# SynthAIr/T-VQ-VAE-TrajGen

Hardware: AMD Instinct MI355X
Metric: stage1+stage2 train steps/sec on synthetic (B,C,T) trajectories, 1/2/4/8 GPU (higher is better)
Workload: dtype fp32; 1 GPU; stage1 VQ-VAE + stage2 MaskGIT joint train step, per-GPU batch (B=256,C=6,T=256), K=512, configs/config.yaml architecture; global_batch=256, seq_len=256, parallelism=dp1, launch=hipgraph

## Files before the change

### include/tvq.h

```cpp
#ifndef TVQ_H
#define TVQ_H
#include <stdint.h>

#ifdef __cplusplus
extern "C" {
#endif

#define TVQ_OK 0
#define TVQ_ERR_ARG -1
#define TVQ_ERR_LAUNCH -2

typedef void* tvq_stream_t;

const char* tvq_last_error(void);
int tvq_abi_version(void);
const char* tvq_source_hash(void);
const char* tvq_build_extra(void);
int tvq_counter_pool(int64_t device, int32_t* zeroed, int64_t n);
int tvq_counter_capture(int64_t begin);
int tvq_fill(float* p, int64_t n, float value, tvq_stream_t stream);
int tvq_fill_i64(int64_t* p, int64_t n, int64_t value, tvq_stream_t stream);
int tvq_fill2(float* p, float a, float* q, float b, tvq_stream_t stream);
int tvq_add_i64(int64_t* p, int64_t value, tvq_stream_t stream);
int tvq_sum4(const float* a, const float* b, const float* c, const float* d, float* out,
// ... 44 lines not shown
                     int32_t* sel, tvq_stream_t stream);

int tvq_vq_expire(const float* x, int64_t B, int64_t N, int64_t D, int64_t sB, int64_t sN,
                  int64_t sD, const int32_t* sel, const int64_t* seed_ptr, uint64_t offset,
                  const float* cluster_size, float threshold, int64_t K, float* embed,
                  int32_t* n_expired, tvq_stream_t stream);

int64_t tvq_vq_kmeans_workspace(int64_t M, int64_t K, int64_t D);
int tvq_vq_kmeans(const float* x, int64_t B, int64_t N, int64_t D, int64_t sB, int64_t sN,
                  int64_t sD, const int32_t* sel, int64_t K, int64_t iters, float* means,
                  float* bins, int32_t* workspace, tvq_stream_t stream);


int tvq_stft_encode(const float* x, int64_t B, int64_t C, int64_t T, float* raw, float* enc_l,
                    float* enc_h, float* tgt_l, float* tgt_h, tvq_stream_t stream);

int tvq_istft_decode(const float* h, int64_t B, int64_t C, int64_t W, int64_t band, int64_t Tout,
                     float* y, tvq_stream_t stream);
int tvq_istft_decode_bwd(const float* dy, int64_t B, int64_t C, int64_t W, int64_t band,
                         int64_t Tout, float* dh, tvq_stream_t stream);

int tvq_conv_out_width(int64_t Win, int64_t KW, int64_t SW, int64_t transposed);
int tvq_conv_config(int64_t halo);

int tvq_conv_packcache_begin(int64_t id, float* arena, int64_t cap_floats, tvq_stream_t stream);
int tvq_conv_packcache_end(void);
int tvq_conv_packcache_release(int64_t id);
int tvq_conv_packcache_pause(int64_t on);
int64_t tvq_conv_packcache_entries(void);

int tvq_conv_wgrad_defer_begin(void);
int tvq_conv_wgrad_defer_flush(tvq_stream_t stream);
int tvq_wgrad_defer_begin_stream(tvq_stream_t stream);
int tvq_conv_wgrad_defer_pause(int64_t paused);
int64_t tvq_conv_workspace(int64_t op, int64_t B, int64_t Ci, int64_t H, int64_t Wi, int64_t Co,
                           int64_t KH, int64_t KW, int64_t SW, int64_t replicate);
int tvq_conv2d_fwd(const float* x, int64_t B, int64_t Ci, int64_t H, int64_t Wi, const float* w,
                   const float* bias, int64_t Co, int64_t KH, int64_t KW, int64_t SW,
                   int64_t replicate, float* y, const float* residual, float drop_p,
                   const int64_t* seed_ptr, uint64_t offset, float* workspace,
                   tvq_stream_t stream);
int tvq_convT2d_fwd(const float* x, int64_t B, int64_t Ci, int64_t H, int64_t Wi, const float* w,
                    const float* bias, int64_t Co, int64_t KH, int64_t KW, int64_t SW, float* y,
                    const float* residual, float* workspace, tvq_stream_t stream);
int tvq_conv2d_fwd_bn_eval(const float* x, int64_t B, int64_t Ci, int64_t H, int64_t Wi,
                           const float* w, const float* bias, int64_t Co, int64_t KH, int64_t KW,
// ... 389 lines not shown
```

### t-vq-vae-trajgen_amd/csrc/tvq_conv.hip

```cpp
#include "tvq_conv_core.h"

namespace tvq {

static ConvConfig g_conv_cfg;
const ConvConfig& conv_config() { return g_conv_cfg; }

__global__ void replicate_fold_kernel(const float* __restrict__ dpad, int B, int C, int H, int W,
                                      int PH, int PW, float* __restrict__ dx) {
  const int Hp = H + 2 * PH, Wp = W + 2 * PW;
  const int64_t tot = (int64_t)B * C * H * W;
  for (int64_t i = blockIdx.x * (int64_t)blockDim.x + threadIdx.x; i < tot;
       i += (int64_t)gridDim.x * blockDim.x) {
    const int w = (int)(i % W);
    const int64_t t = i / W;
    const int h = (int)(t % H);
    const int64_t bc = t / H;
    const float* p = dpad + bc * Hp * Wp;
    const int hlo = h == 0 ? 0 : h + PH, hhi = h == H - 1 ? Hp - 1 : h + PH;
    const int wlo = w == 0 ? 0 : w + PW, whi = w == W - 1 ? Wp - 1 : w + PW;
    float s = 0.f;
    for (int hh = hlo; hh <= hhi; ++hh)
      for (int ww = wlo; ww <= whi; ++ww) s += p[hh * Wp + ww];
    dx[i] = s;
  }
// ... 52 lines not shown
  e.drop_scale = drop_p > 0.f ? 1.0f / (1.0f - drop_p) : 1.0f;
  e.seed_ptr = seed_ptr;
  e.offset = offset;
  return e;
}

extern "C" int tvq_conv_config(int64_t halo) {
  ConvConfig& c = g_conv_cfg;
  const int prev = c.halo | (c.t32 ? 0 : 8) | (c.t32_bk == 32 ? 16 : 0) |
                   (c.t32_bk == 16 ? 32 : 0) | (c.t32_nw == 4 ? 64 : 0) | (c.t32_n64 ? 128 : 0) |
                   (c.small ? 0 : 256) | (c.s2 ? 0 : 512) | (c.ws2 ? 0 : 1024) |
                   (c.n16 ? 0 : 2048);
  if (halo >= 0) {
    c.halo = (int)(halo & 7);
    c.t32 = (halo & 8) ? 0 : 1;
    c.t32_bk = (halo & 16) ? 32 : ((halo & 32) ? 16 : 64);
    c.t32_nw = (halo & 64) ? 4 : 12;
    c.t32_n64 = (halo & 128) ? 1 : 0;
    c.small = (halo & 256) ? 0 : 1;
    c.s2 = (halo & 512) ? 0 : 1;
    c.ws2 = (halo & 1024) ? 0 : 1;
    c.n16 = (halo & 2048) ? 0 : 1;
  }
  return prev;
}

extern "C" int tvq_conv_out_width(int64_t Win, int64_t KW, int64_t SW, int64_t transposed) {
  const int64_t PW = (KW - 1) / 2;
  return (int)(transposed ? (Win - 1) * SW - 2 * PW + KW : (Win + 2 * PW - KW) / SW + 1);
}

static ConvGeom geom_conv_fwd(int64_t B, int64_t Ci, int64_t H, int64_t Wi, int64_t Co, int64_t KH,
                              int64_t KW, int64_t SW) {
  const int Wo = tvq_conv_out_width(Wi, KW, SW, 0);
  return make_geom((int)B, (int)Ci, (int)H, (int)Wi, (int)Co, (int)H, Wo, (int)KH, (int)KW,
                   PH_OF(KH), PW_OF(KW), Ci * KH * KW, KH * KW);
}
static ConvGeom geom_convT_fwd(int64_t B, int64_t Ci, int64_t H, int64_t Wi, int64_t Co,
                               int64_t KH, int64_t KW, int64_t SW) {
  const int Wo = tvq_conv_out_width(Wi, KW, SW, 1);
  return make_geom((int)B, (int)Ci, (int)H, (int)Wi, (int)Co, (int)H, Wo, (int)KH, (int)KW,
                   PH_OF(KH), PW_OF(KW), KH * KW, Co * KH * KW);
}
static ConvGeom geom_conv_dgrad(int64_t B, int64_t Ci, int64_t H, int64_t Wi, int64_t Co,
                                int64_t KH, int64_t KW, int64_t SW, int64_t replicate) {
  const int Wo = tvq_conv_out_width(Wi, KW, SW, 0);
// ... 229 lines not shown
```

### t-vq-vae-trajgen_amd/csrc/tvq_conv_core.h

```cpp
#pragma once
#include "tvq_common.h"

namespace tvq {

struct FastDiv {
  uint32_t d;
  uint64_t magic;
  uint32_t shift;
};
static FastDiv make_fastdiv(uint32_t d) {
  FastDiv f;
  f.d = d;
  uint32_t s = 0;
  while ((1ull << s) < d) ++s;
  f.shift = 32 + s;
  f.magic = ((1ull << f.shift) + d - 1) / d;
  return f;
}
__device__ __forceinline__ uint32_t fdiv(uint32_t n, const FastDiv& f) {
  return (uint32_t)(((uint64_t)n * f.magic) >> f.shift);
}

struct ConvGeom {
  int B, C, Hin, Win;
// ... 249 lines not shown
    switch (kind) {                                                                      \
      case 0: M(GATHER_T, 3, 4, 2, false) break;                                         \
      case 1: M(GATHER_T, 3, 3, 1, false) break;                                         \
      case 2: M(GATHER_T, 1, 1, 1, false) break;                                         \
      case 3: M(GATHER_T, 1, 3, 1, false) break;                                         \
      case 4: M(GATHER_T, 1, 7, 1, false) break;                                         \
      case 5: M(GATHER_T, 1, 4, 2, false) break;                                         \
    }                                                                                    \
  }

#ifndef TVQ_T32_BK
#define TVQ_T32_BK 64
#endif
struct ConvConfig {
  int halo = 3;
  int t32 = 1;
  int t32_bk = TVQ_T32_BK;
  int t32_nw = 12;
  int t32_n64 = 0;
  int small = 1;
  int s2 = 1;
  int ws2 = 1;
  int n16 = 1;
};
const ConvConfig& conv_config();


const float* pack_weight(const float* wt, ConvGeom& g, int KK, float* ws, hipStream_t st);

int s2_kind(int mode, const ConvGeom& g);
int64_t s2_blocks(const ConvGeom& g);
void launch_s2(int k2, bool repl, const float* in, const float* wt, float* out, const ConvGeom& g,
               const Epi& e, hipStream_t st);
bool s2_fold_fits(const ConvGeom& g);
void launch_s2_fold(const float* in, const float* wt, float* dx, const ConvGeom& g, hipStream_t st);
bool ws2_fits(int64_t C, int64_t H, int64_t N, int64_t KH, int64_t KW, int64_t SW);
int64_t ws2_ws(int64_t B, int64_t C, int64_t Wo, int64_t N);
int ws2_launch(const float* G, const float* X, float* slab, int B, int C, int N, int Win, int Wo,
               int kcols, bool repl, hipStream_t st);

bool launch_small(int mode, int kind, bool repl, const float* in, const float* wt, float* out,
                  const ConvGeom& g, const Epi& e, hipStream_t st);
bool n16_geom_ok(int mode, int kind, const ConvGeom& g);
void launch_n16(int mode, int kind, const float* in, const float* wp, float* out,
                const ConvGeom& g, const Epi& e, hipStream_t st);
bool launch_halo(int mode, int kind, bool repl, const float* in, const float* wt, float* out,
// ... 19 lines not shown
```

### t-vq-vae-trajgen_amd/csrc/tvq_conv_s2.hip

```cpp
#include "tvq_conv_core.h"
#include "tvq_reduce.h"

namespace tvq {

constexpr int S2_SEG = 64;
constexpr int S2_XRF = 2 * S2_SEG + 2;
constexpr int S2_XRT = S2_SEG / 2 + 4;

__device__ __forceinline__ void s2_bn_stats_block(double (&s1)[4], double (&s2)[4], int nbase,
                                                  int N, double* __restrict__ part) {
  __shared__ double red[4][16][2];
  const int lane = threadIdx.x & 63, wid = threadIdx.x >> 6;
#pragma unroll
  for (int r = 0; r < 4; ++r)
#pragma unroll
    for (int o = 1; o < 16; o <<= 1) {
      s1[r] += __shfl_xor(s1[r], o, 64);
      s2[r] += __shfl_xor(s2[r], o, 64);
    }
  if ((lane & 15) == 0) {
#pragma unroll
    for (int r = 0; r < 4; ++r) {
      red[wid][nbase + r][0] = s1[r];
      red[wid][nbase + r][1] = s2[r];
    }
  }
  __syncthreads();
  const int t = threadIdx.x;
  if (t < 2 * N) {
    const int n = t >> 1, k = t & 1;
    part[((int64_t)n * gridDim.x + blockIdx.x) * 2 + k] =
        ((red[0][n][k] + red[1][n][k]) + red[2][n][k]) + red[3][n][k];
  }
}

template <bool REPL, int CS, bool POST = false, bool STATS = false>
__global__ __launch_bounds__(256) void conv_s2f_kernel(const float* __restrict__ in,
                                                       const float* __restrict__ wt,
                                                       float* __restrict__ out, ConvGeom g, Epi e) {
  constexpr int NS = 3 * CS, RS = 5;
  constexpr int XN = CS * RS * S2_XRF, XPER = (XN + 255) / 256;
  __shared__ float Xs[XN];
  const int tid = threadIdx.x, lane = tid & 63, r16 = lane & 15, g4 = lane >> 4;
  const int wid = __builtin_amdgcn_readfirstlane(tid >> 6);
  const int segs = (g.Wo + S2_SEG - 1) / S2_SEG;
  const int b = blockIdx.x / segs, w0 = (blockIdx.x - b * segs) * S2_SEG;
  float af[NS];
  const int nr = r16 < g.N ? r16 : 0;
#pragma unroll
  for (int s = 0; s < NS; ++s) {
    const int c = s / 3, kh = s - 3 * c;
    const int cc = c < g.C ? c : 0;
    af[s] = wt[nr * g.wsn + cc * g.wsc + (kh * 4 + g4) * g.wst];
  }
  const float* inb = in + (int64_t)b * g.C * g.Hin * g.Win;
  float xv[XPER];
  uint64_t okm = 0;
#pragma unroll
  for (int u = 0; u < XPER; ++u) {
    const int i = tid + 256 * u;
    const int ck = i / S2_XRF, j = i - ck * S2_XRF, c = ck / RS, r = ck - RS * c;
    int hi = r - 1, wi = 2 * w0 - g.opw + j;
    bool ok = i < XN && c < g.C;
    if (REPL) {
      hi = hi < 0 ? 0 : (hi >= g.Hin ? g.Hin - 1 : hi);
      wi = wi < 0 ? 0 : (wi >= g.Win ? g.Win - 1 : wi);
    } else {
      ok = ok && hi >= 0 && hi < g.Hin && wi >= 0 && wi < g.Win;
    }
    xv[u] = inb[ok ? ((int64_t)c * g.Hin + hi) * g.Win + wi : 0];
    okm |= (uint64_t)(ok ? 1 : 0) << u;
  }
#pragma unroll
  for (int u = 0; u < XPER; ++u) {
    const int i = tid + 256 * u;
    if (i < XN) Xs[i] = (okm >> u & 1) ? xv[u] : 0.f;
  }
  float bv[1][4];
  const int nbase = 4 * g4;
  epi_load_bias<1>(bv, e.bias, nbase, g.N);
  __syncthreads();
  floatx4 acc[3];
  const float* xb[3];
#pragma unroll
  for (int t = 0; t < 3; ++t) {
    const int tile = wid * 3 + t, h = tile >> 2, p0 = (tile & 3) * 16;
    xb[t] = Xs + h * S2_XRF + 2 * (p0 + r16) + g4;
    acc[t] = floatx4{0.f, 0.f, 0.f, 0.f};
  }
#pragma unroll
  for (int s = 0; s < NS; ++s) {
    const int c = s / 3, kh = s - 3 * c, off = (c * RS + kh) * S2_XRF;
#pragma unroll
    for (int t = 0; t < 3; ++t) acc[t] = mfma16x16x4(af[s], xb[t][off], acc[t]);
  }
  const uint64_t seed = e.drop_p > 0.f ? mix_seed(e.seed_ptr, e.offset) : 0ull;
  const int64_t hw = (int64_t)g.Hout * g.Wo;
  PostTile<1> pt;
  if constexpr (POST) epi_load_post<1>(pt, e, nbase, g.N);
#pragma unroll
  for (int t = 0; t < 3; ++t) {
    const int tile = wid * 3 + t, h = tile >> 2;
    const int wo = w0 + (tile & 3) * 16 + r16;
    const bool pv = wo < g.Wo;
    const floatx4 a[1] = {acc[t]};
    epi_store<1, POST>(out, e, seed, bv, a, ((int64_t)b * g.N * g.Hout + h) * g.Wo + (pv ? wo : 0),
                       hw, nbase, g.N, pv, false, &pt);
  }
  if constexpr (STATS) {
    double s1[4] = {0.0, 0.0, 0.0, 0.0}, s2[4] = {0.0, 0.0, 0.0, 0.0};
#pragma unroll
    for (int t = 0; t < 3; ++t) {
      const int tile = wid * 3 + t;
      if (w0 + (tile & 3) * 16 + r16 >= g.Wo) continue;
#pragma unroll
      for (int r = 0; r < 4; ++r) {
        const double v = (double)(acc[t][r] + bv[0][r]);
        s1[r] += v;
        s2[r] += v * v;
      }
    }
    s2_bn_stats_block(s1, s2, nbase, g.N, e.bn_part);
  }
}

template <int CS, int HO, bool FOLD = false, bool POST = false, bool STATS = false>
__global__ __launch_bounds__(256) void conv_s2t_kernel(const float* __restrict__ in,
                                                       const float* __restrict__ wt,
                                                       float* __restrict__ out, ConvGeom g, Epi e) {
  constexpr int NS = 6 * CS / 4, RS = 7;
  constexpr int XN = CS * RS * S2_XRT, XPER = (XN + 255) / 256;
  __shared__ float Xs[XN];
  const int tid = threadIdx.x, lane = tid & 63, r16 = lane & 15, g4 = lane >> 4;
  const int wid = __builtin_amdgcn_readfirstlane(tid >> 6);
  const int par = wid & 1, mb = wid >> 1;
  const int segs = (g.Wo + S2_SEG - 1) / S2_SEG;
  const int b = blockIdx.x / segs, w0 = (blockIdx.x - b * segs) * S2_SEG;
  const int m0 = w0 >> 1;
  float af[NS];
  int soff[NS];
  const int nr = r16 < g.N ? r16 : 0, q = (par + g.opw) & 1;
#pragma unroll
  for (int s = 0; s < NS; ++s) {
    const int k = 4 * s + g4, c = k / 6, rem = k - 6 * c, kh = rem >> 1, kw = q + 2 * (rem & 1);
    const int cc = c < g.C ? c : 0;
    af[s] = wt[nr * g.wsn + cc * g.wsc + (kh * 4 + kw) * g.wst];
    soff[s] = (c * RS - kh) * S2_XRT + ((par + g.opw - kw) >> 1);
  }
  const float* inb = in + (int64_t)b * g.C * g.Hin * g.Win;
  float xv[XPER];
  uint32_t okm = 0;
  static_assert(XPER <= 32, "staging mask");
#pragma unroll
  for (int u = 0; u < XPER; ++u) {
    const int i = tid + 256 * u;
    const int ck = i / S2_XRT, j = i - ck * S2_XRT, c = ck / RS, r = ck - RS * c;
    const int hi = r - 2, wi = m0 - 2 + j;
    const bool ok = i < XN && c < g.C && hi >= 0 && hi < g.Hin && wi >= 0 && wi < g.Win;
    xv[u] = inb[ok ? ((int64_t)c * g.Hin + hi) * g.Win + wi : 0];
    okm |= (uint32_t)(ok ? 1 : 0) << u;
  }
#pragma unroll
  for (int u = 0; u < XPER; ++u) {
    const int i = tid + 256 * u;
    if (i < XN) Xs[i] = (okm >> u & 1) ? xv[u] : 0.f;
  }
  float bv[1][4];
  const int nbase = 4 * g4;
  epi_load_bias<1>(bv, e.bias, nbase, g.N);
  __syncthreads();
  floatx4 acc[HO];
  const float* xb = Xs + (g.oph + 2) * S2_XRT + mb * 16 + r16 + 2;
#pragma unroll
  for (int h = 0; h < HO; ++h) acc[h] = floatx4{0.f, 0.f, 0.f, 0.f};
#pragma unroll
  for (int s = 0; s < NS; ++s)
#pragma unroll
    for (int h = 0; h < HO; ++h) acc[h] = mfma16x16x4(af[s], xb[h * S2_XRT + soff[s]], acc[h]);
  const int wo = w0 + 2 * (mb * 16 + r16) + par;
  if constexpr (FOLD) {
    static_assert(HO == 5, "fold: replicate canvas");
    __shared__ floatx4 ex[2][3][4];
    const int Wx = g.Wo - 2;
    floatx4 y[3] = {acc[0] + acc[1], acc[2], acc[3] + acc[4]};
    if (wo == 0 || wo == Wx + 1) {
#pragma unroll
      for (int h = 0; h < 3; ++h) ex[wo == 0 ? 0 : 1][h][g4] = y[h];
    }
    __syncthreads();
    if (wo == 1) {
#pragma unroll
      for (int h = 0; h < 3; ++h) y[h] = ex[0][h][g4] + y[h];
    } else if (wo == Wx) {
#pragma unroll
      for (int h = 0; h < 3; ++h) y[h] = y[h] + ex[1][h][g4];
    }
    const bool pv = wo >= 1 && wo <= Wx;
#pragma unroll
    for (int h = 0; h < 3; ++h)
#pragma unroll
      for (int r = 0; r < 4; ++r) {
        const int n = nbase + r;
        if (pv && n < g.N) out[(((int64_t)b * g.N + n) * 3 + h) * Wx + wo - 1] = y[h][r];
      }
    return;
  }
  const uint64_t seed = e.drop_p > 0.f ? mix_seed(e.seed_ptr, e.offset) : 0ull;
  const int64_t hw = (int64_t)g.Hout * g.Wo;
  const bool pv = wo < g.Wo;
  PostTile<1> pt;
  if constexpr (POST) epi_load_post<1>(pt, e, nbase, g.N);
#pragma unroll
  for (int h = 0; h < HO; ++h) {
    const floatx4 a[1] = {acc[h]};
    epi_store<1, POST>(out, e, seed, bv, a, ((int64_t)b * g.N * g.Hout + h) * g.Wo + (pv ? wo : 0),
                       hw, nbase, g.N, pv, false, &pt);
  }
  if constexpr (STATS) {
    double s1[4] = {0.0, 0.0, 0.0, 0.0}, s2[4] = {0.0, 0.0, 0.0, 0.0};
    if (pv) {
#pragma unroll
      for (int h = 0; h < HO; ++h)
#pragma unroll
        for (int r = 0; r < 4; ++r) {
          const double v = (double)(acc[h][r] + bv[0][r]);
          s1[r] += v;
          s2[r] += v * v;
        }
    }
    s2_bn_stats_block(s1, s2, nbase, g.N, e.bn_part);
  }
}

int s2_kind(int mode, const ConvGeom& g) {
  if (!conv_config().s2 || g.C > 16 || g.N > 16 || g.Hin != 3) return 0;
  if (mode == GATHER_F)
    return g.Hout == 3 && g.oph == 1 && g.opw >= 0 && g.opw <= 2 ? 1 : 0;
  if (g.opw < 0 || g.opw > 3) return 0;
  if (g.Hout == 3 && g.oph == 1) return 2;
  if (g.Hout == 5 && g.oph == 0) return 3;
  return 0;
}

int64_t s2_blocks(const ConvGeom& g) { return (int64_t)g.B * ((g.Wo + S2_SEG - 1) / S2_SEG); }

template <bool REPL>
static void launch_s2_r(int kind, const float* in, const float* wt, float* out, const ConvGeom& g,
                        const Epi& e, hipStream_t st) {
  const dim3 grid((unsigned)s2_blocks(g));
  const int cs = (g.C + 3) / 4;
  TVQ_PLAN("conv_s2%s cs%d hout%d%s", kind == 1 ? "f" : "t", 4 * cs, g.Hout,
           e.bn_part ? " bnstats" : "");
#define S2F(CSV)                                                                                \
  do {                                                                                          \
    if (e.bn_part)                                                                              \
      hipLaunchKernelGGL((conv_s2f_kernel<REPL, CSV, false, true>), grid, dim3(256), 0, st, in,  \
                         wt, out, g, e);                                                        \
    else if (e.bn_rv)                                                                           \
      hipLaunchKernelGGL((conv_s2f_kernel<REPL, CSV, true>), grid, dim3(256), 0, st, in, wt, out, \
                         g, e);                                                                 \
    else                                                                                        \
      hipLaunchKernelGGL((conv_s2f_kernel<REPL, CSV>), grid, dim3(256), 0, st, in, wt, out, g, e); \
  } while (0)
#define S2T(CSV, HOV)                                                                            \
  do {                                                                                           \
    if (e.bn_part)                                                                               \
      hipLaunchKernelGGL((conv_s2t_kernel<CSV, HOV, false, false, true>), grid, dim3(256), 0, st, \
                         in, wt, out, g, e);                                                     \
    else if (e.bn_rv)                                                                            \
      hipLaunchKernelGGL((conv_s2t_kernel<CSV, HOV, false, true>), grid, dim3(256), 0, st, in, wt, \
                         out, g, e);                                                             \
    else                                                                                         \
      hipLaunchKernelGGL((conv_s2t_kernel<CSV, HOV>), grid, dim3(256), 0, st, in, wt, out, g, e); \
  } while (0)
  if (kind == 1) {
    if (cs == 1) S2F(4); else if (cs == 2) S2F(8); else if (cs == 3) S2F(12); else S2F(16);
    return;
  }
  if (kind == 2) {
    if (cs == 1) S2T(4, 3); else if (cs == 2) S2T(8, 3); else if (cs == 3) S2T(12, 3); else S2T(16, 3);
  } else {
    if (cs == 1) S2T(4, 5); else if (cs == 2) S2T(8, 5); else if (cs == 3) S2T(12, 5); else S2T(16, 5);
  }
#undef S2F
#undef S2T
}
void launch_s2(int k2, bool repl, const float* in, const float* wt, float* out, const ConvGeom& g,
               const Epi& e, hipStream_t st) {
  if (repl) launch_s2_r<true>(k2, in, wt, out, g, e, st);
  else launch_s2_r<false>(k2, in, wt, out, g, e, st);
}

bool s2_fold_fits(const ConvGeom& g) {
  return s2_kind(GATHER_T, g) == 3 && g.Wo >= 4 && (g.Wo - 1) % S2_SEG != 0;
}
void launch_s2_fold(const float* in, const float* wt, float* dx, const ConvGeom& g,
                    hipStream_t st) {
  const dim3 grid((unsigned)s2_blocks(g));
  const Epi e = {nullptr, nullptr, 0.f, 1.f, nullptr, 0};
  const int cs = (g.C + 3) / 4;
  TVQ_PLAN("conv_s2t_fold cs%d", 4 * cs);
#define S2T(CSV) hipLaunchKernelGGL((conv_s2t_kernel<CSV, 5, true>), grid, dim3(256), 0, st, in, wt, dx, g, e)
  if (cs == 1) S2T(4); else if (cs == 2) S2T(8); else if (cs == 3) S2T(12); else S2T(16);
#undef S2T
}

constexpr int W2_T = 512, W2_GS = 3 * S2_SEG + 4, W2_KP = 2 * S2_XRF + 2 * S2_SEG + 8;
struct W2Geom {
  int B, C, N, Win, Wo, Kred, kcols, segs, spr, opw;
};

template <bool REPL, int CS>
__global__ __launch_bounds__(W2_T) void conv_wgrad_s2_kernel(const float* __restrict__ G,
                                                            const float* __restrict__ X,
                                                            float* __restrict__ slab, W2Geom g) {
  constexpr int RS = 5, XN = CS * RS * S2_XRF, XPER = (XN + W2_T - 1) / W2_T;
  constexpr int GN = 16 * 3 * S2_SEG, GPER = GN / W2_T;
  constexpr int KT = (12 * CS + 1 + 15) / 16, TPW = (KT + 3) / 4;
  constexpr int RED = 4 * TPW * 256;
  static_assert(XPER <= 32 && GN % W2_T == 0, "staging");
  __shared__ float Xs[XN > RED ? XN : RED];
  __shared__ float Gs[16 * W2_GS];
  __shared__ float K1[2 * W2_KP];
  const int tid = threadIdx.x, lane = tid & 63, r16 = lane & 15, g4 = lane >> 4;
  const int wid = __builtin_amdgcn_readfirstlane(tid >> 6);
  const int tg = wid & 3, ph = wid >> 2;
  const int nst = g.B * g.segs, z = blockIdx.x;
  const int s_begin = z * g.spr, s_end = min(nst, s_begin + g.spr);
  for (int i = tid; i < 2 * W2_KP; i += W2_T) K1[i] = i < W2_KP ? 1.f : 0.f;
  const float* bp[TPW];
#pragma unroll
  for (int t = 0; t < TPW; ++t) {
    const int kc = (tg + 4 * t) * 16 + r16;
    const int k = kc < g.Kred ? kc : 0, c = k / 12, rem = k - 12 * c, kh = rem >> 2;
    bp[t] = (kc < g.Kred ? Xs + (c * RS + kh) * S2_XRF + (rem & 3)
                         : (kc == g.Kred && g.kcols > g.Kred ? K1 : K1 + W2_KP)) + 2 * g4;
  }
  const float* ap = Gs + r16 * W2_GS + g4;
  float xv[XPER], gv[GPER];
  uint32_t okm = 0, gok = 0;
  auto load = [&](int s) {
    const int b = s / g.segs, w0 = (s - b * g.segs) * S2_SEG;
    const float* xb = X + (int64_t)b * g.C * 3 * g.Win;
#pragma unroll
    for (int u = 0; u < XPER; ++u) {
      const int i = tid + W2_T * u;
      const int ck = i / S2_XRF, j = i - ck * S2_XRF, c = ck / RS, r = ck - RS * c;
      int hi = r - 1, wi = 2 * w0 - g.opw + j;
      bool ok = i < XN && c < g.C;
      if (REPL) {
        hi = hi < 0 ? 0 : (hi > 2 ? 2 : hi);
        wi = wi < 0 ? 0 : (wi >= g.Win ? g.Win - 1 : wi);
      } else {
        ok = ok && hi >= 0 && hi < 3 && wi >= 0 && wi < g.Win;
      }
      xv[u] = xb[ok ? ((int64_t)c * 3 + hi) * g.Win + wi : 0];
      okm = u == 0 ? (ok ? 1u : 0u) : (okm | (ok ? 1u : 0u) << u);
    }
    const float* gb = G + (int64_t)b * g.N * 3 * g.Wo;
#pragma unroll
    for (int u = 0; u < GPER; ++u) {
      const int i = tid + W2_T * u;
      const int n = i / (3 * S2_SEG), p = i - n * (3 * S2_SEG), h = p / S2_SEG, w = w0 + p - h * S2_SEG;
      const bool ok = n < g.N && w < g.Wo;
      gv[u] = gb[ok ? ((int64_t)n * 3 + h) * g.Wo + w : 0];
      gok = u == 0 ? (ok ? 1u : 0u) : (gok | (ok ? 1u : 0u) << u);
    }
  };
  auto store = [&]() {
#pragma unroll
    for (int u = 0; u < XPER; ++u) {
      const int i = tid + W2_T * u;
      if (i < XN) Xs[i] = (okm >> u & 1u) ? xv[u] : 0.f;
    }
#pragma unroll
    for (int u = 0; u < GPER; ++u) {
      const int i = tid + W2_T * u;
      const int n = i / (3 * S2_SEG), p = i - n * (3 * S2_SEG);
      Gs[n * W2_GS + p] = (gok >> u & 1u) ? gv[u] : 0.f;
    }
  };
  floatx4 acc[TPW];
#pragma unroll
  for (int t = 0; t < TPW; ++t) acc[t] = floatx4{0.f, 0.f, 0.f, 0.f};
  if (s_begin < s_end) load(s_begin);
  for (int s = s_begin; s < s_end; ++s) {
    __syncthreads();
    store();
    __syncthreads();
    if (s + 1 < s_end) load(s + 1);
#pragma unroll
    for (int i = 0; i < 24; ++i) {
      const int p0 = 96 * ph + 4 * i, h = p0 / S2_SEG, w = p0 - h * S2_SEG;
      const float a = ap[p0];
      const int off = h * S2_XRF + 2 * w;
#pragma unroll
      for (int t = 0; t < TPW; ++t) acc[t] = mfma16x16x4(a, bp[t][off], acc[t]);
    }
  }
  __syncthreads();
  floatx4* red = reinterpret_cast<floatx4*>(Xs);
  if (ph == 1) {
#pragma unroll
    for (int t = 0; t < TPW; ++t) red[(tg * TPW + t) * 64 + lane] = acc[t];
  }
  __syncthreads();
  if (ph == 0) {
    float* sl = slab + (int64_t)z * g.N * g.kcols;
#pragma unroll
    for (int t = 0; t < TPW; ++t) {
      const floatx4 o = red[(tg * TPW + t) * 64 + lane];
      const int kc = (tg + 4 * t) * 16 + r16;
#pragma unroll
      for (int r = 0; r < 4; ++r) {
        const int n = 4 * g4 + r;
        const float v = acc[t][r] + o[r];
        if (n < g.N && kc < g.kcols) sl[(int64_t)n * g.kcols + kc] = v;
      }
    }
  }
// ... 39 lines not shown
```

### t-vq-vae-trajgen_amd/timevqvae/hip/_native.py

```python
import ctypes
import os
import threading

import torch

_HERE = os.path.dirname(os.path.abspath(__file__))
LIB_PATH = os.environ.get(
    "TVQ_HIP_LIB", os.path.join(os.path.dirname(os.path.dirname(_HERE)), "lib", "libtvq_hip.so"))

P = ctypes.c_void_p
I64 = ctypes.c_int64
I32 = ctypes.c_int
F32 = ctypes.c_float

SIGNATURES = {}
_lib = None
_lock = threading.Lock()


def sig(name, *argtypes, restype=I32):
    SIGNATURES[name] = (list(argtypes), restype)


CSRC = os.path.join(os.path.dirname(os.path.dirname(_HERE)), "csrc")
# ... 48 lines not shown
sig("tvq_vq_sqnorm", P, I64, I64, P, P)
sig("tvq_vq_assign_nblocks", I64, restype=I64)
sig("tvq_vq_assign", P, I64, I64, I64, I64, I64, I64, P, P, I64, I32, P, P, P, P, P)
sig("tvq_vq_stats_workspace", I64, I64, restype=I64)
sig("tvq_vq_stats", P, I64, I64, I64, I64, I64, I64, P, I64, P, P, P, P, P)
sig("tvq_vq_ema", P, P, I64, I64, F32, P, P, P)
sig("tvq_vq_finalize", P, P, I64, I64, F32, P, P, I64, P, P, I64, P, P)
sig("tvq_vq_backward", P, P, P, P, I64, I64, P, P)

U64 = ctypes.c_uint64
sig("tvq_vq_assign_svq", P, I64, I64, I64, I64, I64, I64, P, P, I64, I32, F32, P, P, U64, P, P, P,
    P, P)
sig("tvq_vq_assign_rows", P, I64, I64, I64, I64, I64, I64, P, P, I64, I32, F32, P, P, U64, P, P, P,
    P, P, P)
sig("tvq_vq_draw_rows", I64, I64, P, U64, P, P)
sig("tvq_vq_expire", P, I64, I64, I64, I64, I64, I64, P, P, U64, P, F32, I64, P, P, P)
sig("tvq_vq_kmeans_workspace", I64, I64, I64, restype=I64)
sig("tvq_vq_kmeans", P, I64, I64, I64, I64, I64, I64, P, I64, I64, P, P, P, P)
sig("tvq_stft_encode", P, I64, I64, I64, P, P, P, P, P, P)
sig("tvq_istft_decode", P, I64, I64, I64, I64, I64, P, P)
sig("tvq_istft_decode_bwd", P, I64, I64, I64, I64, I64, P, P)
sig("tvq_conv_out_width", I64, I64, I64, I64)
sig("tvq_conv_config", I64)
sig("tvq_conv_workspace", I64, I64, I64, I64, I64, I64, I64, I64, I64, I64, restype=I64)
sig("tvq_conv2d_fwd", P, I64, I64, I64, I64, P, P, I64, I64, I64, I64, I64, P, P, F32, P, U64, P, P)
sig("tvq_convT2d_fwd", P, I64, I64, I64, I64, P, P, I64, I64, I64, I64, P, P, P, P)
sig("tvq_conv2d_fwd_bn_eval", P, I64, I64, I64, I64, P, P, I64, I64, I64, I64, I64, I64, P, P, P, P,
    F32, P, P, P, P)
sig("tvq_convT2d_fwd_bn_eval", P, I64, I64, I64, I64, P, P, I64, I64, I64, I64, P, P, P, P, F32, P,
    P, P, P)
sig("tvq_conv2d_dgrad", P, I64, I64, I64, I64, P, I64, I64, I64, I64, I64, P, I64, P, P)
sig("tvq_convT2d_dgrad", P, I64, I64, I64, I64, P, I64, I64, I64, I64, P, I64, P, P)
sig("tvq_conv2d_wgrad", P, I64, I64, I64, I64, P, I64, I64, I64, I64, I64, I64, P, P, I64, P, P)
sig("tvq_convT2d_wgrad", P, I64, I64, I64, I64, P, I64, I64, I64, I64, I64, P, I64, P, P)
sig("tvq_channel_sum_workspace", I64, I64, I64, restype=I64)
sig("tvq_channel_sum", P, I64, I64, I64, P, I64, P, P)
sig("tvq_bn_workspace", I64, I64, I64, restype=I64)
sig("tvq_bn_train_fwd", P, I64, I64, I64, P, P, P, P, P, F32, F32, P, P, P, P, P, P, P)
sig("tvq_bn_eval_fwd", P, I64, I64, I64, P, P, P, P, F32, P, P, P, P)
sig("tvq_bn_bwd", P, P, I64, I64, I64, P, P, P, P, P, P, P, P, P, I64, P, P)
sig("tvq_snake_fwd", P, I64, I64, I64, P, P, P)
sig("tvq_snake_workspace", I64, I64, I64, restype=I64)
sig("tvq_snake_bwd", P, P, I64, I64, I64, P, P, P, P, I64, P, P)
sig("tvq_dropout_bwd", P, I64, F32, P, U64, P, P)
sig("tvq_resblock_workspace", I64, I64, I64, I64, restype=I64)
sig("tvq_resblock_saved_floats", I64, I64, I64, I64, restype=I64)
# ... 217 lines not shown
```

Baseline: 260.7 steps/s.

## Make stride-2 conv kernels persistent with double-buffered async global-to-LDS staging

Converts the stride-2 forward and transposed conv kernels from one-segment-per-block into persistent blocks that walk several segments. The next segment is prefetched into a double-buffered dynamic-LDS ring with global_load_lds while the current one runs MFMA. Halo padding rows are no longer staged: only the three real input rows are loaded, and out-of-range rows point at shared zero rows or are clamped through pointer selection. The same row trimming is applied to the stride-2 wgrad kernel. The per-block segment count is controlled by a new s2_cap knob. The aim is to hide load latency and cut redundant staging, at the cost of more LDS, lower occupancy and ring synchronisation overhead.

```diff
diff --git a/include/tvq.h b/include/tvq.h
--- a/include/tvq.h
+++ b/include/tvq.h
@@ -90,6 +90,7 @@
 
 int tvq_conv_out_width(int64_t Win, int64_t KW, int64_t SW, int64_t transposed);
 int tvq_conv_config(int64_t halo);
+int tvq_conv_s2_cap(int64_t cap);
 
 int tvq_conv_packcache_begin(int64_t id, float* arena, int64_t cap_floats, tvq_stream_t stream);
 int tvq_conv_packcache_end(void);
diff --git a/t-vq-vae-trajgen_amd/csrc/tvq_conv.hip b/t-vq-vae-trajgen_amd/csrc/tvq_conv.hip
--- a/t-vq-vae-trajgen_amd/csrc/tvq_conv.hip
+++ b/t-vq-vae-trajgen_amd/csrc/tvq_conv.hip
@@ -98,6 +98,12 @@
     c.ws2 = (halo & 1024) ? 0 : 1;
     c.n16 = (halo & 2048) ? 0 : 1;
   }
+  return prev;
+}
+
+extern "C" int tvq_conv_s2_cap(int64_t cap) {
+  const int prev = g_conv_cfg.s2_cap;
+  if (cap >= 0) g_conv_cfg.s2_cap = cap > (1 << 30) ? (1 << 30) : (int)cap;
   return prev;
 }
 
diff --git a/t-vq-vae-trajgen_amd/csrc/tvq_conv_core.h b/t-vq-vae-trajgen_amd/csrc/tvq_conv_core.h
--- a/t-vq-vae-trajgen_amd/csrc/tvq_conv_core.h
+++ b/t-vq-vae-trajgen_amd/csrc/tvq_conv_core.h
@@ -295,6 +295,7 @@
   int s2 = 1;
   int ws2 = 1;
   int n16 = 1;
+  int s2_cap = 0;
 };
 const ConvConfig& conv_config();
 
diff --git a/t-vq-vae-trajgen_amd/csrc/tvq_conv_s2.hip b/t-vq-vae-trajgen_amd/csrc/tvq_conv_s2.hip
--- a/t-vq-vae-trajgen_amd/csrc/tvq_conv_s2.hip
+++ b/t-vq-vae-trajgen_amd/csrc/tvq_conv_s2.hip
@@ -7,8 +7,25 @@
 constexpr int S2_XRF = 2 * S2_SEG + 2;
 constexpr int S2_XRT = S2_SEG / 2 + 4;
 
+extern __shared__ float s2_lds[];
+static __device__ float s2_zero_word[4];
+
+__device__ __forceinline__ void s2_glds(const float* src, float* dst_wave) {
+  __builtin_amdgcn_global_load_lds((const __attribute__((address_space(1))) void*)src,
+                                   (__attribute__((address_space(3))) void*)dst_wave, 4, 0, 0);
+}
+__device__ __forceinline__ void s2_ring_sync() {
+  asm volatile("s_waitcnt vmcnt(0)" ::: "memory");
+  __syncthreads();
+}
+
+struct S2Run {
+  int nst, spr;
+};
+
 __device__ __forceinline__ void s2_bn_stats_block(double (&s1)[4], double (&s2)[4], int nbase,
-                                                  int N, double* __restrict__ part) {
+                                                  int N, double* __restrict__ part, int slot,
+                                                  int nslots) {
   __shared__ double red[4][16][2];
   const int lane = threadIdx.x & 63, wid = threadIdx.x >> 6;
 #pragma unroll
@@ -29,22 +46,47 @@
   const int t = threadIdx.x;
   if (t < 2 * N) {
     const int n = t >> 1, k = t & 1;
-    part[((int64_t)n * gridDim.x + blockIdx.x) * 2 + k] =
+    part[((int64_t)n * nslots + slot) * 2 + k] =
         ((red[0][n][k] + red[1][n][k]) + red[2][n][k]) + red[3][n][k];
   }
 }
 
+template <int CS>
+struct S2F {
+  static constexpr int RW = CS * S2_XRF;
+  static constexpr int XN = 3 * RW, XNP = (XN + 63) / 64 * 64;
+  static constexpr int XPER = (XNP + 255) / 256;
+  static int lds_bytes(bool repl, int nbuf) { return (nbuf * XNP + (repl ? 0 : RW)) * 4; }
+};
 template <bool REPL, int CS, bool POST = false, bool STATS = false>
 __global__ __launch_bounds__(256) void conv_s2f_kernel(const float* __restrict__ in,
                                                        const float* __restrict__ wt,
-                                                       float* __restrict__ out, ConvGeom g, Epi e) {
-  constexpr int NS = 3 * CS, RS = 5;
-  constexpr int XN = CS * RS * S2_XRF, XPER = (XN + 255) / 256;
-  __shared__ float Xs[XN];
+                                                       float* __restrict__ out, ConvGeom g, Epi e,
+                                                       S2Run run) {
+  using L = S2F<CS>;
+  constexpr int NS = 3 * CS;
+  float* const Xs = s2_lds;
   const int tid = threadIdx.x, lane = tid & 63, r16 = lane & 15, g4 = lane >> 4;
   const int wid = __builtin_amdgcn_readfirstlane(tid >> 6);
   const int segs = (g.Wo + S2_SEG - 1) / S2_SEG;
-  const int b = blockIdx.x / segs, w0 = (blockIdx.x - b * segs) * S2_SEG;
+  const int s_begin = blockIdx.x * run.spr, s_end = min(run.nst, s_begin + run.spr);
+  float* const Zs = Xs + (run.spr > 1 ? 2 : 1) * L::XNP;
+  auto stage = [&](int st, float* buf) {
+    const int b = st / segs, w0 = (st - b * segs) * S2_SEG;
+    const float* inb = in + (int64_t)b * g.C * 3 * g.Win;
+#pragma unroll
+    for (int u = 0; u < L::XPER; ++u) {
+      if (256 * u + 64 * wid >= L::XNP) break;
+      const int i = tid + 256 * u;
+      const int rc = i / S2_XRF, j = i - rc * S2_XRF, r = rc / CS, c = rc - r * CS;
+      int wi = 2 * w0 - g.opw + j;
+      bool ok = i < L::XN && c < g.C;
+      if (REPL) wi = wi < 0 ? 0 : (wi >= g.Win ? g.Win - 1 : wi);
+      else ok = ok && wi >= 0 && wi < g.Win;
+      s2_glds(ok ? inb + ((int64_t)c * 3 + r) * g.Win + wi : s2_zero_word, buf + 256 * u + 64 * wid);
+    }
+  };
+  stage(s_begin, Xs);
   float af[NS];
   const int nr = r16 < g.N ? r16 : 0;
 #pragma unroll
@@ -53,90 +95,105 @@
     const int cc = c < g.C ? c : 0;
     af[s] = wt[nr * g.wsn + cc * g.wsc + (kh * 4 + g4) * g.wst];
   }
-  const float* inb = in + (int64_t)b * g.C * g.Hin * g.Win;
-  float xv[XPER];
-  uint64_t okm = 0;
-#pragma unroll
-  for (int u = 0; u < XPER; ++u) {
-    const int i = tid + 256 * u;
-    const int ck = i / S2_XRF, j = i - ck * S2_XRF, c = ck / RS, r = ck - RS * c;
-    int hi = r - 1, wi = 2 * w0 - g.opw + j;
-    bool ok = i < XN && c < g.C;
-    if (REPL) {
-      hi = hi < 0 ? 0 : (hi >= g.Hin ? g.Hin - 1 : hi);
-      wi = wi < 0 ? 0 : (wi >= g.Win ? g.Win - 1 : wi);
-    } else {
-      ok = ok && hi >= 0 && hi < g.Hin && wi >= 0 && wi < g.Win;
-    }
-    xv[u] = inb[ok ? ((int64_t)c * g.Hin + hi) * g.Win + wi : 0];
-    okm |= (uint64_t)(ok ? 1 : 0) << u;
-  }
-#pragma unroll
-  for (int u = 0; u < XPER; ++u) {
-    const int i = tid + 256 * u;
-    if (i < XN) Xs[i] = (okm >> u & 1) ? xv[u] : 0.f;
-  }
   float bv[1][4];
   const int nbase = 4 * g4;
   epi_load_bias<1>(bv, e.bias, nbase, g.N);
-  __syncthreads();
-  floatx4 acc[3];
-  const float* xb[3];
-#pragma unroll
-  for (int t = 0; t < 3; ++t) {
-    const int tile = wid * 3 + t, h = tile >> 2, p0 = (tile & 3) * 16;
-    xb[t] = Xs + h * S2_XRF + 2 * (p0 + r16) + g4;
-    acc[t] = floatx4{0.f, 0.f, 0.f, 0.f};
-  }
-#pragma unroll
-  for (int s = 0; s < NS; ++s) {
-    const int c = s / 3, kh = s - 3 * c, off = (c * RS + kh) * S2_XRF;
-#pragma unroll
-    for (int t = 0; t < 3; ++t) acc[t] = mfma16x16x4(af[s], xb[t][off], acc[t]);
-  }
   const uint64_t seed = e.drop_p > 0.f ? mix_seed(e.seed_ptr, e.offset) : 0ull;
   const int64_t hw = (int64_t)g.Hout * g.Wo;
   PostTile<1> pt;
   if constexpr (POST) epi_load_post<1>(pt, e, nbase, g.N);
-#pragma unroll
-  for (int t = 0; t < 3; ++t) {
-    const int tile = wid * 3 + t, h = tile >> 2;
-    const int wo = w0 + (tile & 3) * 16 + r16;
-    const bool pv = wo < g.Wo;
-    const floatx4 a[1] = {acc[t]};
-    epi_store<1, POST>(out, e, seed, bv, a, ((int64_t)b * g.N * g.Hout + h) * g.Wo + (pv ? wo : 0),
-                       hw, nbase, g.N, pv, false, &pt);
-  }
-  if constexpr (STATS) {
-    double s1[4] = {0.0, 0.0, 0.0, 0.0}, s2[4] = {0.0, 0.0, 0.0, 0.0};
+  if (!REPL)
+    for (int i = tid; i < L::RW; i += 256) Zs[i] = 0.f;
+  for (int st = s_begin; st < s_end; ++st) {
+    float* const cur = Xs + ((st - s_begin) & 1) * L::XNP;
+    s2_ring_sync();
+    if (st + 1 < s_end) stage(st + 1, Xs + ((st + 1 - s_begin) & 1) * L::XNP);
+    const int b = st / segs, w0 = (st - b * segs) * S2_SEG;
+    floatx4 acc[3];
+    const float* rb[3][3];
 #pragma unroll
     for (int t = 0; t < 3; ++t) {
-      const int tile = wid * 3 + t;
-      if (w0 + (tile & 3) * 16 + r16 >= g.Wo) continue;
-#pragma unroll
-      for (int r = 0; r < 4; ++r) {
-        const double v = (double)(acc[t][r] + bv[0][r]);
-        s1[r] += v;
-        s2[r] += v * v;
-      }
-    }
-    s2_bn_stats_block(s1, s2, nbase, g.N, e.bn_part);
-  }
-}
-
+      const int tile = wid * 3 + t, h = tile >> 2, p0 = (tile & 3) * 16;
+      const int col = 2 * (p0 + r16) + g4;
+#pragma unroll
+      for (int kh = 0; kh < 3; ++kh) {
+        const int hi = h + kh - 1;
+        if (REPL) rb[t][kh] = cur + (hi < 0 ? 0 : (hi > 2 ? 2 : hi)) * L::RW + col;
+        else rb[t][kh] = (hi >= 0 && hi <= 2 ? cur + hi * L::RW : Zs) + col;
+      }
+      acc[t] = floatx4{0.f, 0.f, 0.f, 0.f};
+    }
+#pragma unroll
+    for (int s = 0; s < NS; ++s) {
+      const int c = s / 3, kh = s - 3 * c;
+#pragma unroll
+      for (int t = 0; t < 3; ++t) acc[t] = mfma16x16x4(af[s], rb[t][kh][c * S2_XRF], acc[t]);
+    }
+#pragma unroll
+    for (int t = 0; t < 3; ++t) {
+      const int tile = wid * 3 + t, h = tile >> 2;
+      const int wo = w0 + (tile & 3) * 16 + r16;
+      const bool pv = wo < g.Wo;
+      const floatx4 a[1] = {acc[t]};
+      epi_store<1, POST>(out, e, seed, bv, a, ((int64_t)b * g.N * g.Hout + h) * g.Wo + (pv ? wo : 0),
+                         hw, nbase, g.N, pv, false, &pt);
+    }
+    if constexpr (STATS) {
+      double s1[4] = {0.0, 0.0, 0.0, 0.0}, s2[4] = {0.0, 0.0, 0.0, 0.0};
+#pragma unroll
+      for (int t = 0; t < 3; ++t) {
+        const int tile = wid * 3 + t;
+        if (w0 + (tile & 3) * 16 + r16 >= g.Wo) continue;
+#pragma unroll
+        for (int r = 0; r < 4; ++r) {
+          const double v = (double)(acc[t][r] + bv[0][r]);
+          s1[r] += v;
+          s2[r] += v * v;
+        }
+      }
+      s2_bn_stats_block(s1, s2, nbase, g.N, e.bn_part, st, run.nst);
+    }
+  }
+}
+
+template <int CS, int HO>
+struct S2T {
+  static constexpr int ZR = HO == 5 ? 2 : 1;
+  static constexpr int RW = CS * S2_XRT;
+  static constexpr int XN = 3 * RW, XNP = (XN + 63) / 64 * 64;
+  static constexpr int XPER = (XNP + 255) / 256;
+  static constexpr int PER = (3 + ZR) * RW;
+  static_assert(XNP - XN <= ZR * RW, "the DMA's tail must stay inside the zeros");
+  static int lds_bytes(int nbuf) { return (nbuf * PER + ZR * RW) * 4; }
+};
 template <int CS, int HO, bool FOLD = false, bool POST = false, bool STATS = false>
 __global__ __launch_bounds__(256) void conv_s2t_kernel(const float* __restrict__ in,
                                                        const float* __restrict__ wt,
-                                                       float* __restrict__ out, ConvGeom g, Epi e) {
-  constexpr int NS = 6 * CS / 4, RS = 7;
-  constexpr int XN = CS * RS * S2_XRT, XPER = (XN + 255) / 256;
-  __shared__ float Xs[XN];
+                                                       float* __restrict__ out, ConvGeom g, Epi e,
+                                                       S2Run run) {
+  using L = S2T<CS, HO>;
+  constexpr int NS = 6 * CS / 4;
+  float* const Xs = s2_lds;
   const int tid = threadIdx.x, lane = tid & 63, r16 = lane & 15, g4 = lane >> 4;
   const int wid = __builtin_amdgcn_readfirstlane(tid >> 6);
   const int par = wid & 1, mb = wid >> 1;
   const int segs = (g.Wo + S2_SEG - 1) / S2_SEG;
-  const int b = blockIdx.x / segs, w0 = (blockIdx.x - b * segs) * S2_SEG;
-  const int m0 = w0 >> 1;
+  const int s_begin = blockIdx.x * run.spr, s_end = min(run.nst, s_begin + run.spr);
+  const int nbuf = run.spr > 1 ? 2 : 1;
+  auto stage = [&](int st, float* buf) {
+    const int b = st / segs, m0 = ((st - b * segs) * S2_SEG) >> 1;
+    const float* inb = in + (int64_t)b * g.C * 3 * g.Win;
+#pragma unroll
+    for (int u = 0; u < L::XPER; ++u) {
+      if (256 * u + 64 * wid >= L::XNP) break;
+      const int i = tid + 256 * u;
+      const int rc = i / S2_XRT, j = i - rc * S2_XRT, r = rc / CS, c = rc - r * CS;
+      const int wi = m0 - 2 + j;
+      const bool ok = i < L::XN && c < g.C && wi >= 0 && wi < g.Win;
+      s2_glds(ok ? inb + ((int64_t)c * 3 + r) * g.Win + wi : s2_zero_word, buf + 256 * u + 64 * wid);
+    }
+  };
+  stage(s_begin, Xs + L::ZR * L::RW);
   float af[NS];
   int soff[NS];
   const int nr = r16 < g.N ? r16 : 0, q = (par + g.opw) & 1;
@@ -145,90 +202,80 @@
     const int k = 4 * s + g4, c = k / 6, rem = k - 6 * c, kh = rem >> 1, kw = q + 2 * (rem & 1);
     const int cc = c < g.C ? c : 0;
     af[s] = wt[nr * g.wsn + cc * g.wsc + (kh * 4 + kw) * g.wst];
-    soff[s] = (c * RS - kh) * S2_XRT + ((par + g.opw - kw) >> 1);
-  }
-  const float* inb = in + (int64_t)b * g.C * g.Hin * g.Win;
-  float xv[XPER];
-  uint32_t okm = 0;
-  static_assert(XPER <= 32, "staging mask");
-#pragma unroll
-  for (int u = 0; u < XPER; ++u) {
-    const int i = tid + 256 * u;
-    const int ck = i / S2_XRT, j = i - ck * S2_XRT, c = ck / RS, r = ck - RS * c;
-    const int hi = r - 2, wi = m0 - 2 + j;
-    const bool ok = i < XN && c < g.C && hi >= 0 && hi < g.Hin && wi >= 0 && wi < g.Win;
-    xv[u] = inb[ok ? ((int64_t)c * g.Hin + hi) * g.Win + wi : 0];
-    okm |= (uint32_t)(ok ? 1 : 0) << u;
-  }
-#pragma unroll
-  for (int u = 0; u < XPER; ++u) {
-    const int i = tid + 256 * u;
-    if (i < XN) Xs[i] = (okm >> u & 1) ? xv[u] : 0.f;
+    soff[s] = (c - kh * CS) * S2_XRT + ((par + g.opw - kw) >> 1);
   }
   float bv[1][4];
   const int nbase = 4 * g4;
   epi_load_bias<1>(bv, e.bias, nbase, g.N);
-  __syncthreads();
-  floatx4 acc[HO];
-  const float* xb = Xs + (g.oph + 2) * S2_XRT + mb * 16 + r16 + 2;
-#pragma unroll
-  for (int h = 0; h < HO; ++h) acc[h] = floatx4{0.f, 0.f, 0.f, 0.f};
-#pragma unroll
-  for (int s = 0; s < NS; ++s)
-#pragma unroll
-    for (int h = 0; h < HO; ++h) acc[h] = mfma16x16x4(af[s], xb[h * S2_XRT + soff[s]], acc[h]);
-  const int wo = w0 + 2 * (mb * 16 + r16) + par;
-  if constexpr (FOLD) {
-    static_assert(HO == 5, "fold: replicate canvas");
-    __shared__ floatx4 ex[2][3][4];
-    const int Wx = g.Wo - 2;
-    floatx4 y[3] = {acc[0] + acc[1], acc[2], acc[3] + acc[4]};
-    if (wo == 0 || wo == Wx + 1) {
-#pragma unroll
-      for (int h = 0; h < 3; ++h) ex[wo == 0 ? 0 : 1][h][g4] = y[h];
-    }
-    __syncthreads();
-    if (wo == 1) {
-#pragma unroll
-      for (int h = 0; h < 3; ++h) y[h] = ex[0][h][g4] + y[h];
-    } else if (wo == Wx) {
-#pragma unroll
-      for (int h = 0; h < 3; ++h) y[h] = y[h] + ex[1][h][g4];
-    }
-    const bool pv = wo >= 1 && wo <= Wx;
-#pragma unroll
-    for (int h = 0; h < 3; ++h)
-#pragma unroll
-      for (int r = 0; r < 4; ++r) {
-        const int n = nbase + r;
-        if (pv && n < g.N) out[(((int64_t)b * g.N + n) * 3 + h) * Wx + wo - 1] = y[h][r];
-      }
-    return;
-  }
   const uint64_t seed = e.drop_p > 0.f ? mix_seed(e.seed_ptr, e.offset) : 0ull;
   const int64_t hw = (int64_t)g.Hout * g.Wo;
-  const bool pv = wo < g.Wo;
   PostTile<1> pt;
   if constexpr (POST) epi_load_post<1>(pt, e, nbase, g.N);
-#pragma unroll
-  for (int h = 0; h < HO; ++h) {
-    const floatx4 a[1] = {acc[h]};
-    epi_store<1, POST>(out, e, seed, bv, a, ((int64_t)b * g.N * g.Hout + h) * g.Wo + (pv ? wo : 0),
-                       hw, nbase, g.N, pv, false, &pt);
-  }
-  if constexpr (STATS) {
-    double s1[4] = {0.0, 0.0, 0.0, 0.0}, s2[4] = {0.0, 0.0, 0.0, 0.0};
-    if (pv) {
-#pragma unroll
-      for (int h = 0; h < HO; ++h)
+  for (int i = tid; i < nbuf * L::PER + L::ZR * L::RW; i += 256)
+    if ((i / L::RW) % (3 + L::ZR) < L::ZR) Xs[i] = 0.f;
+  for (int st = s_begin; st < s_end; ++st) {
+    float* const cur = Xs + ((st - s_begin) & 1) * L::PER;
+    s2_ring_sync();
+    if (st + 1 < s_end) stage(st + 1, Xs + ((st + 1 - s_begin) & 1) * L::PER + L::ZR * L::RW);
+    const int b = st / segs, w0 = (st - b * segs) * S2_SEG;
+    floatx4 acc[HO];
+    const float* xb = cur + (g.oph + L::ZR) * L::RW + mb * 16 + r16 + 2;
+#pragma unroll
+    for (int h = 0; h < HO; ++h) acc[h] = floatx4{0.f, 0.f, 0.f, 0.f};
+#pragma unroll
+    for (int s = 0; s < NS; ++s)
+#pragma unroll
+      for (int h = 0; h < HO; ++h) acc[h] = mfma16x16x4(af[s], xb[h * L::RW + soff[s]], acc[h]);
+    const int wo = w0 + 2 * (mb * 16 + r16) + par;
+    if constexpr (FOLD) {
+      static_assert(HO == 5, "fold: replicate canvas");
+      __shared__ floatx4 ex[2][3][4];
+      const int Wx = g.Wo - 2;
+      floatx4 y[3] = {acc[0] + acc[1], acc[2], acc[3] + acc[4]};
+      if (wo == 0 || wo == Wx + 1) {
+#pragma unroll
+        for (int h = 0; h < 3; ++h) ex[wo == 0 ? 0 : 1][h][g4] = y[h];
+      }
+      __syncthreads();
+      if (wo == 1) {
+#pragma unroll
+        for (int h = 0; h < 3; ++h) y[h] = ex[0][h][g4] + y[h];
+      } else if (wo == Wx) {
+#pragma unroll
+        for (int h = 0; h < 3; ++h) y[h] = y[h] + ex[1][h][g4];
+      }
+      const bool pv = wo >= 1 && wo <= Wx;
+#pragma unroll
+      for (int h = 0; h < 3; ++h)
 #pragma unroll
         for (int r = 0; r < 4; ++r) {
-          const double v = (double)(acc[h][r] + bv[0][r]);
-          s1[r] += v;
-          s2[r] += v * v;
+          const int n = nbase + r;
+          if (pv && n < g.N) out[(((int64_t)b * g.N + n) * 3 + h) * Wx + wo - 1] = y[h][r];
         }
-    }
-    s2_bn_stats_block(s1, s2, nbase, g.N, e.bn_part);
+    } else {
+      const bool pv = wo < g.Wo;
+#pragma unroll
+      for (int h = 0; h < HO; ++h) {
+        const floatx4 a[1] = {acc[h]};
+        epi_store<1, POST>(out, e, seed, bv, a,
+                           ((int64_t)b * g.N * g.Hout + h) * g.Wo + (pv ? wo : 0), hw, nbase, g.N,
+                           pv, false, &pt);
+      }
+      if constexpr (STATS) {
+        double s1[4] = {0.0, 0.0, 0.0, 0.0}, s2[4] = {0.0, 0.0, 0.0, 0.0};
+        if (pv) {
+#pragma unroll
+          for (int h = 0; h < HO; ++h)
+#pragma unroll
+            for (int r = 0; r < 4; ++r) {
+              const double v = (double)(acc[h][r] + bv[0][r]);
+              s1[r] += v;
+              s2[r] += v * v;
+            }
+        }
+        s2_bn_stats_block(s1, s2, nbase, g.N, e.bn_part, st, run.nst);
+      }
+    }
   }
 }
 
@@ -244,34 +291,53 @@
 
 int64_t s2_blocks(const ConvGeom& g) { return (int64_t)g.B * ((g.Wo + S2_SEG - 1) / S2_SEG); }
 
+constexpr int S2_CAP_DEFAULT = 768;
+static S2Run s2_run(const ConvGeom& g, unsigned* grid) {
+  const int64_t nst = s2_blocks(g);
+  const int64_t cap = conv_config().s2_cap > 0 ? conv_config().s2_cap : S2_CAP_DEFAULT;
+  const int64_t blocks = nst < cap ? nst : cap;
+  S2Run r;
+  r.nst = (int)nst;
+  r.spr = (int)((nst + blocks - 1) / blocks);
+  *grid = (unsigned)((nst + r.spr - 1) / r.spr);
+  return r;
+}
+
 template <bool REPL>
 static void launch_s2_r(int kind, const float* in, const float* wt, float* out, const ConvGeom& g,
                         const Epi& e, hipStream_t st) {
-  const dim3 grid((unsigned)s2_blocks(g));
+  unsigned blocks;
+  const S2Run run = s2_run(g, &blocks);
+  const dim3 grid(blocks);
+  const int nbuf = run.spr > 1 ? 2 : 1;
   const int cs = (g.C + 3) / 4;
-  TVQ_PLAN("conv_s2%s cs%d hout%d%s", kind == 1 ? "f" : "t", 4 * cs, g.Hout,
-           e.bn_part ? " bnstats" : "");
-#define S2F(CSV)                                                                                \
-  do {                                                                                          \
-    if (e.bn_part)                                                                              \
-      hipLaunchKernelGGL((conv_s2f_kernel<REPL, CSV, false, true>), grid, dim3(256), 0, st, in,  \
-                         wt, out, g, e);                                                        \
-    else if (e.bn_rv)                                                                           \
-      hipLaunchKernelGGL((conv_s2f_kernel<REPL, CSV, true>), grid, dim3(256), 0, st, in, wt, out, \
-                         g, e);                                                                 \
-    else                                                                                        \
-      hipLaunchKernelGGL((conv_s2f_kernel<REPL, CSV>), grid, dim3(256), 0, st, in, wt, out, g, e); \
+  TVQ_PLAN("conv_s2%s cs%d hout%d%s blocks=%u per=%d", kind == 1 ? "f" : "t", 4 * cs, g.Hout,
+           e.bn_part ? " bnstats" : "", blocks, run.spr);
+#define S2F(CSV)                                                                                  \
+  do {                                                                                            \
+    const int lds = S2F<CSV>::lds_bytes(REPL, nbuf);                                              \
+    if (e.bn_part)                                                                                \
+      hipLaunchKernelGGL((conv_s2f_kernel<REPL, CSV, false, true>), grid, dim3(256), lds, st, in,  \
+                         wt, out, g, e, run);                                                     \
+    else if (e.bn_rv)                                                                             \
+      hipLaunchKernelGGL((conv_s2f_kernel<REPL, CSV, true>), grid, dim3(256), lds, st, in, wt,     \
+                         out, g, e, run);                                                         \
+    else                                                                                          \
+      hipLaunchKernelGGL((conv_s2f_kernel<REPL, CSV>), grid, dim3(256), lds, st, in, wt, out, g,   \
+                         e, run);                                                                 \
   } while (0)
-#define S2T(CSV, HOV)                                                                            \
-  do {                                                                                           \
-    if (e.bn_part)                                                                               \
-      hipLaunchKernelGGL((conv_s2t_kernel<CSV, HOV, false, false, true>), grid, dim3(256), 0, st, \
-                         in, wt, out, g, e);                                                     \
-    else if (e.bn_rv)                                                                            \
-      hipLaunchKernelGGL((conv_s2t_kernel<CSV, HOV, false, true>), grid, dim3(256), 0, st, in, wt, \
-                         out, g, e);                                                             \
-    else                                                                                         \
-      hipLaunchKernelGGL((conv_s2t_kernel<CSV, HOV>), grid, dim3(256), 0, st, in, wt, out, g, e); \
+#define S2T(CSV, HOV)                                                                              \
+  do {                                                                                             \
+    const int lds = S2T<CSV, HOV>::lds_bytes(nbuf);                                                \
+    if (e.bn_part)                                                                                 \
+      hipLaunchKernelGGL((conv_s2t_kernel<CSV, HOV, false, false, true>), grid, dim3(256), lds, st, \
+                         in, wt, out, g, e, run);                                                  \
+    else if (e.bn_rv)                                                                              \
+      hipLaunchKernelGGL((conv_s2t_kernel<CSV, HOV, false, true>), grid, dim3(256), lds, st, in,    \
+                         wt, out, g, e, run);                                                      \
+    else                                                                                           \
+      hipLaunchKernelGGL((conv_s2t_kernel<CSV, HOV>), grid, dim3(256), lds, st, in, wt, out, g, e,  \
+                         run);                                                                     \
   } while (0)
   if (kind == 1) {
     if (cs == 1) S2F(4); else if (cs == 2) S2F(8); else if (cs == 3) S2F(12); else S2F(16);
@@ -296,11 +362,16 @@
 }
 void launch_s2_fold(const float* in, const float* wt, float* dx, const ConvGeom& g,
                     hipStream_t st) {
-  const dim3 grid((unsigned)s2_blocks(g));
+  unsigned blocks;
+  const S2Run run = s2_run(g, &blocks);
+  const dim3 grid(blocks);
+  const int nbuf = run.spr > 1 ? 2 : 1;
   const Epi e = {nullptr, nullptr, 0.f, 1.f, nullptr, 0};
   const int cs = (g.C + 3) / 4;
-  TVQ_PLAN("conv_s2t_fold cs%d", 4 * cs);
-#define S2T(CSV) hipLaunchKernelGGL((conv_s2t_kernel<CSV, 5, true>), grid, dim3(256), 0, st, in, wt, dx, g, e)
+  TVQ_PLAN("conv_s2t_fold cs%d blocks=%u per=%d", 4 * cs, blocks, run.spr);
+#define S2T(CSV)                                                                            \
+  hipLaunchKernelGGL((conv_s2t_kernel<CSV, 5, true>), grid, dim3(256),                      \
+                     (S2T<CSV, 5>::lds_bytes(nbuf)), st, in, wt, dx, g, e, run)
   if (cs == 1) S2T(4); else if (cs == 2) S2T(8); else if (cs == 3) S2T(12); else S2T(16);
 #undef S2T
 }
@@ -314,7 +385,7 @@
 __global__ __launch_bounds__(W2_T) void conv_wgrad_s2_kernel(const float* __restrict__ G,
                                                             const float* __restrict__ X,
                                                             float* __restrict__ slab, W2Geom g) {
-  constexpr int RS = 5, XN = CS * RS * S2_XRF, XPER = (XN + W2_T - 1) / W2_T;
+  constexpr int RS = 3, XN = CS * RS * S2_XRF, XPER = (XN + W2_T - 1) / W2_T;
   constexpr int GN = 16 * 3 * S2_SEG, GPER = GN / W2_T;
   constexpr int KT = (12 * CS + 1 + 15) / 16, TPW = (KT + 3) / 4;
   constexpr int RED = 4 * TPW * 256;
@@ -328,13 +399,22 @@
   const int nst = g.B * g.segs, z = blockIdx.x;
   const int s_begin = z * g.spr, s_end = min(nst, s_begin + g.spr);
   for (int i = tid; i < 2 * W2_KP; i += W2_T) K1[i] = i < W2_KP ? 1.f : 0.f;
-  const float* bp[TPW];
+  const float* bp[3][TPW];
 #pragma unroll
   for (int t = 0; t < TPW; ++t) {
     const int kc = (tg + 4 * t) * 16 + r16;
     const int k = kc < g.Kred ? kc : 0, c = k / 12, rem = k - 12 * c, kh = rem >> 2;
-    bp[t] = (kc < g.Kred ? Xs + (c * RS + kh) * S2_XRF + (rem & 3)
-                         : (kc == g.Kred && g.kcols > g.Kred ? K1 : K1 + W2_KP)) + 2 * g4;
+    const float* plane = (kc == g.Kred && g.kcols > g.Kred ? K1 : K1 + W2_KP) + 2 * g4;
+    auto row = [&](int h) -> const float* {
+      if (kc >= g.Kred) return plane;
+      int hi = h + kh - 1;
+      if (REPL) hi = hi < 0 ? 0 : (hi > 2 ? 2 : hi);
+      else if (hi < 0 || hi > 2) return K1 + W2_KP + 2 * g4;
+      return Xs + (c * RS + hi) * S2_XRF + (rem & 3) + 2 * g4;
+    };
+    bp[0][t] = row(ph) + 64 * ph;
+    bp[1][t] = row(2 * ph) - 64 * ph;
+    bp[2][t] = row(ph + 1) + 64 * ph - 128;
   }
   const float* ap = Gs + r16 * W2_GS + g4;
   float xv[XPER], gv[GPER];
@@ -345,15 +425,11 @@
 #pragma unroll
     for (int u = 0; u < XPER; ++u) {
       const int i = tid + W2_T * u;
-      const int ck = i / S2_XRF, j = i - ck * S2_XRF, c = ck / RS, r = ck - RS * c;
-      int hi = r - 1, wi = 2 * w0 - g.opw + j;
+      const int ck = i / S2_XRF, j = i - ck * S2_XRF, c = ck / RS, hi = ck - RS * c;
+      int wi = 2 * w0 - g.opw + j;
       bool ok = i < XN && c < g.C;
-      if (REPL) {
-        hi = hi < 0 ? 0 : (hi > 2 ? 2 : hi);
-        wi = wi < 0 ? 0 : (wi >= g.Win ? g.Win - 1 : wi);
-      } else {
-        ok = ok && hi >= 0 && hi < 3 && wi >= 0 && wi < g.Win;
-      }
+      if (REPL) wi = wi < 0 ? 0 : (wi >= g.Win ? g.Win - 1 : wi);
+      else ok = ok && wi >= 0 && wi < g.Win;
       xv[u] = xb[ok ? ((int64_t)c * 3 + hi) * g.Win + wi : 0];
       okm = u == 0 ? (ok ? 1u : 0u) : (okm | (ok ? 1u : 0u) << u);
     }
@@ -391,11 +467,9 @@
     if (s + 1 < s_end) load(s + 1);
 #pragma unroll
     for (int i = 0; i < 24; ++i) {
-      const int p0 = 96 * ph + 4 * i, h = p0 / S2_SEG, w = p0 - h * S2_SEG;
-      const float a = ap[p0];
-      const int off = h * S2_XRF + 2 * w;
-#pragma unroll
-      for (int t = 0; t < TPW; ++t) acc[t] = mfma16x16x4(a, bp[t][off], acc[t]);
+      const float a = ap[96 * ph + 4 * i];
+#pragma unroll
+      for (int t = 0; t < TPW; ++t) acc[t] = mfma16x16x4(a, bp[i >> 3][t][8 * i], acc[t]);
     }
   }
   __syncthreads();
diff --git a/t-vq-vae-trajgen_amd/timevqvae/hip/_native.py b/t-vq-vae-trajgen_amd/timevqvae/hip/_native.py
--- a/t-vq-vae-trajgen_amd/timevqvae/hip/_native.py
+++ b/t-vq-vae-trajgen_amd/timevqvae/hip/_native.py
@@ -94,6 +94,7 @@
 sig("tvq_istft_decode_bwd", P, I64, I64, I64, I64, I64, P, P)
 sig("tvq_conv_out_width", I64, I64, I64, I64)
 sig("tvq_conv_config", I64)
+sig("tvq_conv_s2_cap", I64)
 sig("tvq_conv_workspace", I64, I64, I64, I64, I64, I64, I64, I64, I64, I64, restype=I64)
 sig("tvq_conv2d_fwd", P, I64, I64, I64, I64, P, P, I64, I64, I64, I64, I64, P, P, F32, P, U64, P, P)
 sig("tvq_convT2d_fwd", P, I64, I64, I64, I64, P, P, I64, I64, I64, I64, P, P, P, P)
```

New measurement: 263.9 steps/s, median of 6. +1.2%, better.
